# tsy935/eeg-gnn-ssl

Hardware: AMD Instinct MI355X
Metric: EEG clips/sec (60s, 19ch, K=2, 2-layer x64) fwd+bwd (higher is better)
Workload: dtype f32

## Files before the change

### eeg_gnn_ssl_amd/csrc/kernels_gemm_f.h

```cpp
#pragma once
#include "common.h"
#include "kernels_gemm_q.h"
#include "spec_launch.h"

namespace eeg {


__host__ __device__ constexpr int tnf_ndma(int FXT) { return (kTnfRC / 8) * (FXT + 10); }
__host__ __device__ constexpr int tnf_per(int FXT) { return (tnf_ndma(FXT) + 3) / 4; }

template <int FXT>
struct TnfRing {
    static constexpr int PER = tnf_per(FXT);
    const wbuf_t (&dsc)[PER];
    const int (&lofs)[PER];
    const unsigned (&vof)[PER];
    unsigned (&soff)[PER];
    const unsigned (&cstep)[PER];
};
template <int FXT, class LoadF, class MmaF>
__device__ __forceinline__ void tnf_ring(float* sm, const int Q, const TnfRing<FXT>& rg, LoadF load, MmaF mma) {
    constexpr int RC = kTnfRC, NS = tnf_ns(FXT), KS = RC / 2, PER = tnf_per(FXT), ST = tnf_stage_floats(FXT);
    int d_stage = 0;
    auto issue = [&]() __attribute__((always_inline)) {
        float* base = sm + d_stage * ST;
#pragma unroll
        for (int j = 0; j < PER; ++j) {
            wbuf_dma16(rg.dsc[j], base + rg.lofs[j], rg.vof[j], rg.soff[j]);
            rg.soff[j] += rg.cstep[j];
        }
        d_stage = d_stage + 1 == NS ? 0 : d_stage + 1;
    };
#pragma unroll
    for (int p = 0; p < NS - 1; ++p)
        if (p < Q) issue();
    int r_stage = 0;
    for (int q = 0; q < Q; ++q) {
        if (q + NS - 1 <= Q) vm_wait_barrier_n<(NS - 2) * PER>();
        else EEG_VM_WAIT_BARRIER(0);
#ifndef EEG_X_TNF_NODMA
        if (q + NS - 1 < Q) issue();
#endif
        const float* st = sm + r_stage * ST;
        load(IntC<0>(), st, 0);
#pragma unroll
        for (int ks = 0; ks < KS; ++ks) {
            if (ks & 1) {
                if (ks + 1 < KS) load(IntC<0>(), st, ks + 1);
                EEG_SCHED_FENCE();
                mma(IntC<1>());
            } else {
                if (ks + 1 < KS) load(IntC<1>(), st, ks + 1);
                EEG_SCHED_FENCE();
                mma(IntC<0>());
            }
            EEG_SCHED_FENCE();
        }
        r_stage = r_stage + 1 == NS ? 0 : r_stage + 1;
    }
}
__device__ __forceinline__ void tnf_store_tile(float* __restrict__ out, int ld, int f0, int c0, int fmax, int lane, const f32x16& t) {
    const int hh = lane >> 5, l32 = lane & 31;
#pragma unroll
    for (int v = 0; v < 16; ++v) {
        const int f = f0 + 8 * (v >> 2) + 4 * hh + (v & 3);
        if (f < fmax) out[(size_t)f * ld + c0 + l32] = t[v];
    }
}

template <int FXT, int S>
__device__ __forceinline__ void tnf_role(float* sm, const int Q, const int Fin, const int e, const int lane, const TnfRing<FXT>& rg,
                                         float* __restrict__ px, float* __restrict__ pg, float* __restrict__ pc) {
    constexpr int RC = kTnfRC, NXT = (FXT + 1) / 2;
    constexpr int RM = RC / 8, HI = RM * FXT * 256, RI = HI + RM * 512, YI = RI + RM * 512;
    constexpr int YX = 3 * S, YE = S == 0 ? 4 : 2;
    const int hh = lane >> 5, l32 = lane & 31;
    f32x16 ax[NXT][3], ah[2], ar;
#pragma unroll
    for (int v = 0; v < 16; ++v) {
#pragma unroll
        for (int a = 0; a < NXT; ++a)
#pragma unroll
            for (int c = 0; c < 3; ++c) ax[a][c][v] = 0.f;
        ah[0][v] = 0.f; ah[1][v] = 0.f; ar[v] = 0.f;
    }
    const int ox = hh * Fin + 32 * e + l32, oh = HI + hh * 64 + 32 * e + l32, orr = RI + hh * 64 + 32 * e + l32, oy = YI + hh * 192 + l32;
    float fx[2][NXT], fh[2], fr[2], fy[2][4];
    auto load = [&](auto PAR, const float* st, int ks) __attribute__((always_inline)) {
        constexpr int p = decltype(PAR)::value;
#pragma unroll
        for (int a = 0; a < NXT; ++a) fx[p][a] = st[ox + 2 * ks * Fin + 64 * a];
        fh[p] = st[oh + 2 * ks * 64];
        fr[p] = st[orr + 2 * ks * 64];
#pragma unroll
        for (int c = 0; c < 3; ++c) fy[p][c] = st[oy + 2 * ks * 192 + 32 * (YX + c)];
        fy[p][3] = st[oy + 2 * ks * 192 + 32 * YE];
    };
    auto mma = [&](auto PAR) __attribute__((always_inline)) {
        constexpr int p = decltype(PAR)::value;
#pragma unroll
        for (int a = 0; a < NXT; ++a)
#pragma unroll
#ifndef EEG_X_TNF_NOMFMA
            for (int c = 0; c < 3; ++c) ax[a][c] = mfma32(fx[p][a], fy[p][c], ax[a][c]);
#else
            for (int c = 0; c < 3; ++c) ax[a][c][0] += fx[p][a] * fy[p][c];
#endif
#ifndef EEG_X_TNF_NOMFMA
        ah[0] = mfma32(fh[p], S == 0 ? fy[p][0] : fy[p][3], ah[0]);
        ah[1] = mfma32(fh[p], S == 0 ? fy[p][1] : fy[p][0], ah[1]);
        ar = mfma32(fr[p], S == 0 ? fy[p][3] : fy[p][2], ar);
#else
        ah[0][0] += fh[p] * (S == 0 ? fy[p][0] : fy[p][3]);
        ah[1][0] += fh[p] * (S == 0 ? fy[p][1] : fy[p][0]);
        ar[0] += fr[p] * (S == 0 ? fy[p][3] : fy[p][2]);
#endif
    };
    tnf_ring<FXT>(sm, Q, rg, load, mma);
#pragma unroll
    for (int a = 0; a < NXT; ++a) {
        const int xe = e + 2 * a;
        if (xe >= FXT) continue;
#pragma unroll
        for (int c = 0; c < 3; ++c) tnf_store_tile(px, 192, 32 * xe, 32 * (YX + c), Fin, lane, ax[a][c]);
    }
    tnf_store_tile(pg, 128, 32 * e, 32 * (2 * S), 64, lane, ah[0]);
    tnf_store_tile(pg, 128, 32 * e, 32 * (2 * S + 1), 64, lane, ah[1]);
    tnf_store_tile(pc, 64, 32 * e, 32 * S, 64, lane, ar);
}

template <int S, int E>
__device__ __forceinline__ void tnf_role_r4(float* sm, const int Q, const int lane, const TnfRing<4>& rg,
                                            float* __restrict__ px, float* __restrict__ pg, float* __restrict__ pc) {
    constexpr int FXT = 4, Fin = 100, RC = kTnfRC, RM = RC / 8, HI = RM * FXT * 256, RI = HI + RM * 512, YI = RI + RM * 512;
    constexpr int YX = 3 * S, YE = S == 0 ? 4 : 2, NG = S == 0 ? 2 : 1, G0 = S == 0 ? 0 : 2;
    const int hh = lane >> 5, l32 = lane & 31;
    f32x16 t[8];
    f32x4 rem[2];
#pragma unroll
    for (int i = 0; i < 8; ++i)
#pragma unroll
        for (int v = 0; v < 16; ++v) t[i][v] = 0.f;
    rem[0] = rem[1] = (f32x4){0.f, 0.f, 0.f, 0.f};
    const int oxa = hh * Fin + (E == 0 ? 0 : 32) + l32, oxb = hh * Fin + 64 + l32;
    const int oh = HI + hh * 64 + 32 * E + l32, or0 = RI + hh * 64 + l32, oy = YI + hh * 192 + l32;
    const int oxr = 96 + (lane & 3), oyr = YI + lane;
    float fa[2][4], fy[2][4], ra[2][2], rb[2][2][2];
    auto load = [&](auto PAR, const float* st, int ks) __attribute__((always_inline)) {
        constexpr int p = decltype(PAR)::value;
        fa[p][0] = st[oxa + 2 * ks * Fin];
        fa[p][1] = st[E == 0 ? oxb + 2 * ks * Fin : oh + 2 * ks * 64];
        if (E == 0) fa[p][2] = st[oh + 2 * ks * 64];
        else { fa[p][2] = st[or0 + 2 * ks * 64]; fa[p][3] = st[or0 + 32 + 2 * ks * 64]; }
#pragma unroll
        for (int c = 0; c < 3; ++c) fy[p][c] = st[oy + 2 * ks * 192 + 32 * (YX + c)];
        if (E == 1 || S == 1) fy[p][3] = st[oy + 2 * ks * 192 + 32 * YE];
        if (E == 1) {
#pragma unroll
            for (int r = 0; r < 2; ++r) {
                ra[p][r] = st[(2 * ks + r) * Fin + oxr];
#pragma unroll
                for (int g = 0; g < NG; ++g) rb[p][r][g] = st[oyr + (2 * ks + r) * 192 + 64 * (G0 + g)];
            }
        }
    };
    auto mma = [&](auto PAR) __attribute__((always_inline)) {
        constexpr int p = decltype(PAR)::value;
        const float g0 = S == 0 ? fy[p][0] : fy[p][3], g1 = S == 0 ? fy[p][1] : fy[p][0];
#pragma unroll
        for (int c = 0; c < 3; ++c) t[c] = mfma32(fa[p][0], fy[p][c], t[c]);
        if (E == 0) {
#pragma unroll
            for (int c = 0; c < 3; ++c) t[3 + c] = mfma32(fa[p][1], fy[p][c], t[3 + c]);
            t[6] = mfma32(fa[p][2], g0, t[6]);
            t[7] = mfma32(fa[p][2], g1, t[7]);
        } else {
            const float cd = S == 0 ? fy[p][3] : fy[p][2];
            t[3] = mfma32(fa[p][1], g0, t[3]);
            t[4] = mfma32(fa[p][1], g1, t[4]);
            t[5] = mfma32(fa[p][2], cd, t[5]);
            t[6] = mfma32(fa[p][3], cd, t[6]);
#pragma unroll
            for (int r = 0; r < 2; ++r)
#pragma unroll
                for (int g = 0; g < NG; ++g) rem[g] = mfma4(ra[p][r], rb[p][r][g], rem[g]);
        }
    };
    tnf_ring<4>(sm, Q, rg, load, mma);
    if (E == 0) {
#pragma unroll
        for (int c = 0; c < 3; ++c) {
            tnf_store_tile(px, 192, 0, 32 * (YX + c), Fin, lane, t[c]);
            tnf_store_tile(px, 192, 64, 32 * (YX + c), Fin, lane, t[3 + c]);
        }
        tnf_store_tile(pg, 128, 0, 32 * (2 * S), 64, lane, t[6]);
        tnf_store_tile(pg, 128, 0, 32 * (2 * S + 1), 64, lane, t[7]);
    } else {
#pragma unroll
        for (int c = 0; c < 3; ++c) tnf_store_tile(px, 192, 32, 32 * (YX + c), Fin, lane, t[c]);
        tnf_store_tile(pg, 128, 32, 32 * (2 * S), 64, lane, t[3]);
        tnf_store_tile(pg, 128, 32, 32 * (2 * S + 1), 64, lane, t[4]);
        tnf_store_tile(pc, 64, 0, 32 * S, 64, lane, t[5]);
        tnf_store_tile(pc, 64, 32, 32 * S, 64, lane, t[6]);
#pragma unroll
        for (int g = 0; g < NG; ++g)
#pragma unroll
            for (int r = 0; r < 4; ++r) px[(size_t)(96 + r) * 192 + 64 * (G0 + g) + lane] = rem[g][r];
    }
}

template <int FXT>
__global__ __launch_bounds__(256, tnf_wgs_per_cu(FXT)) void gemm_tnf_kernel(const float* __restrict__ Xh, long long x_gstride, int Fin,
                                                         const float* __restrict__ Hh, long long h_gstride,
                                                         const float* __restrict__ RHh, const float* __restrict__ dY, int Sp, int spg, int rps,
                                                         float* __restrict__ part_x, float* __restrict__ part_g, float* __restrict__ part_c) {
    constexpr int RC = kTnfRC, RM = RC / 8, NDMA = tnf_ndma(FXT), PER = tnf_per(FXT), NX = RM * FXT, NH = RM * 2;
    constexpr int HI = NX * 256, RI = HI + NH * 256, YI = RI + NH * 256;
    EEG_DYN_SMEM(sm);
    const int tid = threadIdx.x, lane = tid & 63, w = wave_uniform(tid >> 6), e = w & 1, s = w >> 1;
    const int y = (int)blockIdx.x, i = y / spg, ls = y - i * spg;
    const int rbeg = ls * rps;
    int rend = rbeg + rps;
    if (rend > Sp) rend = Sp;
    const int Q = rend > rbeg ? (rend - rbeg) / RC : 0;
    wbuf_t dsc[PER];
    int lofs[PER];
    unsigned vof[PER], soff[PER], cstep[PER];
    const wbuf_t rx = make_wbuf(Xh + (size_t)i * x_gstride), rh = make_wbuf(Hh + (size_t)i * h_gstride);
    const wbuf_t rr = make_wbuf(RHh + (size_t)i * Sp * 64), ry = make_wbuf(dY + (size_t)i * Sp * 192);
#pragma unroll
    for (int j = 0; j < PER; ++j) {
        int d = w + 4 * j;
        if (d >= NDMA) d = NDMA - 1;
        if (d < NX) {
            dsc[j] = rx; lofs[j] = d * 256; cstep[j] = (unsigned)(RC * Fin) * 4u;
            soff[j] = (unsigned)(rbeg * Fin) * 4u;
            vof[j] = d * 1024 + lane * 16 < RC * Fin * 4 ? (unsigned)(d * 1024 + lane * 16) : 0u;
        } else if (d < NX + NH) {
            dsc[j] = rh; lofs[j] = HI + (d - NX) * 256; cstep[j] = RC * 64 * 4u;
            soff[j] = (unsigned)(rbeg * 64) * 4u; vof[j] = (unsigned)((d - NX) * 1024 + lane * 16);
        } else if (d < NX + 2 * NH) {
            dsc[j] = rr; lofs[j] = RI + (d - NX - NH) * 256; cstep[j] = RC * 64 * 4u;
            soff[j] = (unsigned)(rbeg * 64) * 4u; vof[j] = (unsigned)((d - NX - NH) * 1024 + lane * 16);
        } else {
            dsc[j] = ry; lofs[j] = YI + (d - NX - 2 * NH) * 256; cstep[j] = RC * 192 * 4u;
            soff[j] = (unsigned)(rbeg * 192) * 4u; vof[j] = (unsigned)((d - NX - 2 * NH) * 1024 + lane * 16);
        }
    }
    float* px = part_x + (size_t)y * Fin * 192;
    float* pg = part_g + (size_t)y * 64 * 128;
    float* pc = part_c + (size_t)y * 64 * 64;
    const TnfRing<FXT> rg{dsc, lofs, vof, soff, cstep};
#ifndef EEG_X_TNF_NOR4
    if constexpr (FXT == 4) {
        if (Fin == 100) {
            if (s == 0) { if (e == 0) tnf_role_r4<0, 0>(sm, Q, lane, rg, px, pg, pc); else tnf_role_r4<0, 1>(sm, Q, lane, rg, px, pg, pc); }
            else { if (e == 0) tnf_role_r4<1, 0>(sm, Q, lane, rg, px, pg, pc); else tnf_role_r4<1, 1>(sm, Q, lane, rg, px, pg, pc); }
            return;
        }
    }
#endif
    if (s == 0) tnf_role<FXT, 0>(sm, Q, Fin, e, lane, rg, px, pg, pc);
    else tnf_role<FXT, 1>(sm, Q, Fin, e, lane, rg, px, pg, pc);
}

template <int KQ, bool SWZ>
__global__ __launch_bounds__(256, 2) void gemm_nnf_kernel(const float* __restrict__ A, long long a_gstride, int K, int Sp, int G,
                                                         const float* __restrict__ Wr, unsigned w_gstride, float* __restrict__ C,
                                                         const float* __restrict__ bias, const float* __restrict__ gscale) {
    constexpr int NS = kNnfNS;
    EEG_DYN_SMEM(sm);
    const int tid = threadIdx.x, lane = tid & 63, w = wave_uniform(tid >> 6), rw = w & 1, cw = w >> 1, hh = lane >> 5, l32 = lane & 31;
    const int ST = nnf_stage_floats(K), CPG = ceil_div(Sp, 64), total = G * CPG;
    const int NPC = ceil_div(64 * K, 256), PER = ceil_div(NPC, 4);
    const int g0 = (int)(((long long)blockIdx.x * total) / gridDim.x), g1 = (int)(((long long)(blockIdx.x + 1) * total) / gridDim.x);
    const int Q = g1 - g0;
    if (tid < 4 * NS) sm[(tid >> 2) * ST + 64 * K + (tid & 3)] = 0.f;
    const unsigned lane_src = SWZ ? (unsigned)((lane >> 4) * 256 + (((lane & 15) ^ ((4 * w + (lane >> 4)) & 15)) << 4)) : (unsigned)lane * 16u;
    int d_g = g0, d_stage = 0, d_grp = -1;
    wbuf_t ra = make_wbuf_n(A, 0u);
    auto issue = [&]() __attribute__((always_inline)) {
        const int grp = d_g / CPG, lc = d_g - grp * CPG;
        if (grp != d_grp) { d_grp = grp; ra = make_wbuf_n(A + (size_t)grp * a_gstride, (unsigned)(Sp * K) * 4u); }
        float* base = sm + d_stage * ST;
        const unsigned cb = (unsigned)(lc * 64 * K) * 4u;
        for (int j = 0; j < PER; ++j) {
            int p = w + 4 * j;
            if (p >= NPC) p = NPC - 1;
            wbuf_dma16(ra, base + p * 256, cb + (unsigned)p * 1024u + lane_src, 0u);
        }
        d_stage = d_stage + 1 == NS ? 0 : d_stage + 1;
        ++d_g;
    };
    float wr[KQ][4][3];
    f32x16 acc[3];
    float binit[3] = {0.f, 0.f, 0.f};
    int c_grp = -1;
    wbuf_t rc = make_wbuf_n(C, 0u);
    const int row = 32 * rw + l32;
    const int a_row = row * K;
    const int ccol = 32 * 3 * cw + l32;
#pragma unroll 1
    for (int p = 0; p < NS - 1; ++p)
        if (p < Q) issue();
    int r_stage = 0;
#pragma unroll 1
    for (int q = 0; q < Q; ++q) {
        const int g = g0 + q, grp = g / CPG, lc = g - grp * CPG;
        if (grp != c_grp) {
            c_grp = grp;
            const wbuf_t rwt = make_wbuf(Wr + (size_t)grp * w_gstride);
#pragma unroll
            for (int kq = 0; kq < KQ; ++kq)
#pragma unroll
                for (int s = 0; s < 4; ++s)
#pragma unroll
                    for (int t = 0; t < 3; ++t) wr[kq][s][t] = wbuf_ld(rwt, (unsigned)(4 * hh * 192 + ccol), (unsigned)((8 * kq + s) * 192 + 32 * t));
            const float gs = bias != nullptr ? gscale[grp] : 0.f;
#pragma unroll
            for (int t = 0; t < 3; ++t) binit[t] = bias != nullptr ? gs * bias[ccol + 32 * t] : 0.f;
            rc = make_wbuf_n(C + (size_t)grp * Sp * 192, (unsigned)(Sp * 192) * 4u);
        }
        {
            int nd = Q - 1 - q;
            if (nd > NS - 2) nd = NS - 2;
            const int n = 48 * (q < NS - 1 ? q : NS - 1) + PER * nd;
            if (n >= 63) vm_wait_n<63>(); else if (n >= 55) vm_wait_n<55>(); else if (n >= 52) vm_wait_n<52>(); else if (n >= 48) vm_wait_n<48>();
            else if (n >= 14) vm_wait_n<14>(); else if (n >= 8) vm_wait_n<8>(); else if (n >= 7) vm_wait_n<7>(); else if (n >= 4) vm_wait_n<4>();
            else vm_wait_n<0>();
        }
#ifndef EEG_X_NNF_NOBAR
        EEG_LDS_BARRIER();
#endif
#ifndef EEG_X_NNF_NODMA
        if (q + NS - 1 < Q) issue();
#endif
        const float* st = sm + r_stage * ST;
#pragma unroll
        for (int t = 0; t < 3; ++t)
#pragma unroll
            for (int v = 0; v < 16; ++v) acc[t][v] = binit[t];
        f32x4 a4 = *reinterpret_cast<const f32x4*>(st + a_row + (SWZ ? ((hh ^ (row & 15)) << 2) : 4 * hh));
#pragma unroll
        for (int kq = 0; kq < KQ; ++kq) {
            f32x4 an = a4;
#ifndef EEG_X_NNF_NOLDS
            if (kq + 1 < KQ) an = *reinterpret_cast<const f32x4*>(st + a_row + (SWZ ? (((2 * (kq + 1) + hh) ^ (row & 15)) << 2) : 4 * (2 * (kq + 1) + hh)));
#endif
            EEG_SCHED_FENCE();
#pragma unroll
            for (int s = 0; s < 4; ++s)
#pragma unroll
                for (int t = 0; t < 3; ++t) acc[t] = mfma32(a4[s], wr[kq][s][t], acc[t]);
            EEG_SCHED_FENCE();
            a4 = an;
        }
        unsigned ob[4];
#pragma unroll
        for (int b = 0; b < 4; ++b) {
            ob[b] = (unsigned)((lc * 64 + 32 * rw + 4 * hh + 8 * b) * 192 + ccol);
            EEG_PIN(ob[b]);
        }
#pragma unroll
        for (int t = 0; t < 3; ++t)
#pragma unroll
#ifndef EEG_X_NNF_NOSTORE
            for (int v = 0; v < 16; ++v) wbuf_st1(rc, ob[v >> 2] + (unsigned)((v & 3) * 192 + 32 * t), 0u, acc[t][v]);
#else
            for (int v = 0; v < 16; ++v) { EEG_USE(acc[t][v]); (void)rc; }
#endif
        EEG_SCHED_FENCE();
        r_stage = r_stage + 1 == NS ? 0 : r_stage + 1;
    }
}


template <int NT>
__global__ __launch_bounds__(256, 2) void gemm_dxf_kernel(const float* __restrict__ dYh, int Sp, int S, int Nrt, const float* __restrict__ Wtq,
                                                         unsigned w_gstride, const float* __restrict__ basis, float* __restrict__ dX) {
    const int N = NT > 0 ? NT : Nrt;
    constexpr int NS = kDxfNS, ST = kDxfStage, RB = kDxfRows, PER = 6;
    EEG_DYN_SMEM(sm);
    const int tid = threadIdx.x, lane = tid & 63, w = wave_uniform(tid >> 6), lr = lane & 15, lg = lane >> 4;
    const int r0 = (int)blockIdx.x * RB;
    unsigned src[PER];
#pragma unroll
    for (int j = 0; j < PER; ++j) {
        const int P = 64 * (w + 4 * j) + lane, row = P / 48, slot = P - row * 48;
        const int unit = (slot & ~15) | ((slot & 15) ^ (row & 15));
        src[j] = (unsigned)((r0 + row) * 768 + unit * 16);
    }
    int d_i = 0, d_stage = 0;
    auto issue = [&]() __attribute__((always_inline)) {
        const wbuf_t ra = make_wbuf_n(dYh + (size_t)d_i * Sp * 192, (unsigned)(Sp * 192) * 4u);
        float* base = sm + d_stage * ST;
#pragma unroll
        for (int j = 0; j < PER; ++j) wbuf_dma16(ra, base + (w + 4 * j) * 256, src[j], 0u);
        d_stage = d_stage + 1 == NS ? 0 : d_stage + 1;
        if (d_i + 1 < N) ++d_i;
    };
    f32x4 acc[kDxfMaxN][2];
#pragma unroll
    for (int j = 0; j < kDxfMaxN; ++j) acc[j][0] = acc[j][1] = (f32x4){0.f, 0.f, 0.f, 0.f};
    f32x4 wq[12];
    const unsigned wl = (unsigned)(w * 64 + lane) * 4u;
    static_assert(kDxfNS == 3, "the queue discipline below is written for two images in flight");
    issue();
    issue();
    EEG_SCHED_FENCE();
    {
        const wbuf_t rw0 = make_wbuf(Wtq);
#pragma unroll
        for (int c = 0; c < 12; ++c) wq[c] = wbuf_ld4(rw0, wl, (unsigned)(c * 4 * 256));
    }
    vm_wait_n<PER + 12>();
    int r_stage = 0;
    const int a_row = lr * 192;
#pragma unroll 1
    for (int i = 0; i < N; ++i) {
        EEG_LDS_BARRIER();
#ifndef EEG_X_DXF_NODMA
        issue();
#endif
        const wbuf_t rwn = make_wbuf(Wtq + (size_t)(i + 1 < N ? i + 1 : i) * w_gstride);
        const float* st = sm + r_stage * ST;
        float uu[kDxfMaxN];
#pragma unroll
        for (int j = 0; j < kDxfMaxN; ++j) uu[j] = (NT > 0 ? j < NT : j < N) ? basis[j * N + i] : 0.f;
        f32x4 t0 = {0.f, 0.f, 0.f, 0.f}, t1 = {0.f, 0.f, 0.f, 0.f};
        auto frag_off = [&](int c) __attribute__((always_inline)) {
            const int u = 4 * c + lg;
            return a_row + (((u & ~15) | ((u & 15) ^ lr)) << 2);
        };
        f32x4 fa[2][2];
        fa[0][0] = *reinterpret_cast<const f32x4*>(st + frag_off(0));
        fa[0][1] = *reinterpret_cast<const f32x4*>(st + 16 * 192 + frag_off(0));
#pragma unroll
        for (int c = 0; c < 12; ++c) {
            if (c + 1 < 12) {
                fa[(c + 1) & 1][0] = *reinterpret_cast<const f32x4*>(st + frag_off(c + 1));
                fa[(c + 1) & 1][1] = *reinterpret_cast<const f32x4*>(st + 16 * 192 + frag_off(c + 1));
            }
            EEG_SCHED_FENCE();
#pragma unroll
            for (int e = 0; e < 4; ++e) {
                t0 = mfma16(wq[c][e], fa[c & 1][0][e], t0);
                t1 = mfma16(wq[c][e], fa[c & 1][1][e], t1);
            }
            EEG_SCHED_FENCE();
#ifndef EEG_X_DXF_NOW
            wq[c] = wbuf_ld4(rwn, wl, (unsigned)(c * 4 * 256));
#endif
            EEG_SCHED_FENCE();
        }
#pragma unroll
        for (int j = 0; j < kDxfMaxN; ++j)
            if (NT > 0 ? j < NT : j < N) {
                acc[j][0] += t0 * uu[j];
                acc[j][1] += t1 * uu[j];
            }
        r_stage = r_stage + 1 == NS ? 0 : r_stage + 1;
    }
    const wbuf_t rx = make_wbuf_n(dX, (unsigned)(S * N * 64) * 4u);
#pragma unroll
    for (int t = 0; t < 2; ++t) {
        const unsigned rb = (unsigned)((r0 + 16 * t + lr) * N * 64 + 16 * w + 4 * lg);
#pragma unroll
        for (int j = 0; j < kDxfMaxN; ++j)
            if (j < N) wbuf_st4(rx, rb + (unsigned)(j * 64), 0u, acc[j][t]);
    }
}

}
```

### eeg_gnn_ssl_amd/csrc/spec_common.h

```cpp
#pragma once
#include "common.h"
#include "nnq_order.h"

namespace eeg {

constexpr int kSpecTc = kMaxM * 32, kSpecInfo = 32, kSpecCsum = 32;
__host__ __device__ constexpr int spec_basis_floats(int N) { return N * N + kSpecTc + kSpecInfo + kSpecCsum; }
__host__ __device__ constexpr int spec_csum_offset(int N) { return N * N + kSpecTc + kSpecInfo; }
__host__ __device__ constexpr int spec_rows(int S) { return round_up(S, 16); }
constexpr int kSpecSweeps = 12;

struct SpecPack {
    int Fin, H, M, N;
    int nch_x, nct_x, nch_t, nct_t;
    size_t sxq, sxq_stride, sxtq, sxtq_stride, sxr, sxr_stride, total;
};
__host__ __device__ inline SpecPack make_spec_pack(int Fin, int H, int M, int N) {
    SpecPack p;
    p.Fin = Fin; p.H = H; p.M = M; p.N = N;
    p.nch_x = make_nnq_order(1, Fin).nch; p.nct_x = 3 * H / 16;
    p.nch_t = make_nnq_order(1, 3 * H).nch; p.nct_t = round_up(Fin, 16) / 16;
    p.sxq_stride = (size_t)p.nch_x * p.nct_x * 256;
    p.sxtq_stride = (size_t)p.nch_t * p.nct_t * 256;
    p.sxq = 0;
    p.sxtq = p.sxq + p.sxq_stride * N;
    p.sxr = p.sxtq + p.sxtq_stride * N;
    p.sxr_stride = (size_t)round_up(Fin, 8) * 3 * H;
    p.total = p.sxr + p.sxr_stride * N;
    return p;
}
struct SpecFoldJob {
    const float* part;
    int spg, K, O, nblocks;
};
struct SpecFoldJobs {
    SpecFoldJob j[3];
    const float* basis;
    int N;
};
__host__ __device__ inline size_t spec_fold_lds_bytes(int M, int nsplit_max) { return 256 * 16 + (size_t)M * nsplit_max * sizeof(float); }
template <int MM>
__device__ __forceinline__ void spec_fold_block_m(int block, const SpecFoldJob& jb, int kind, const float* __restrict__ basis, int N,
                                                   int acc_flag, int Fin, int H, int M, float* __restrict__ dWg, float* __restrict__ dWc) {
    EEG_DYN_SMEM(sm);
    float4 (*red)[16] = reinterpret_cast<float4 (*)[16]>(sm);
    float* tcl = sm + 256 * 4;
    const int O = jb.O;
    const size_t total = (size_t)jb.K * O;
    const int g = threadIdx.x >> 4, q = threadIdx.x & 15;
    const size_t idx4 = ((size_t)block * 16 + q) * 4;
    const float* tc = basis + N * N;
    const int nsplit = N * jb.spg;
    for (int e = threadIdx.x; e < M * nsplit; e += 256) {
        const int m = e / nsplit, sp = e - m * nsplit;
        tcl[e] = tc[m * 32 + sp / jb.spg];
    }
    __syncthreads();
    float4 a[MM];
#pragma unroll
    for (int m = 0; m < MM; ++m) a[m] = make_float4(0.f, 0.f, 0.f, 0.f);
    if (idx4 < total) {
        constexpr int UN = 8;
        for (int base = g; base < nsplit; base += 16 * UN) {
            float4 v[UN];
#pragma unroll
            for (int u = 0; u < UN; ++u) {
                const int sp = base + 16 * u;
                v[u] = sp < nsplit ? *reinterpret_cast<const float4*>(jb.part + (size_t)sp * total + idx4) : make_float4(0.f, 0.f, 0.f, 0.f);
            }
#pragma unroll
            for (int u = 0; u < UN; ++u) {
                const int sp = base + 16 * u < nsplit ? base + 16 * u : 0;
#pragma unroll
                for (int m = 0; m < MM; ++m) {
                    if (m < M) {
                        const float t = tcl[m * nsplit + sp];
                        a[m].x = fmaf(t, v[u].x, a[m].x); a[m].y = fmaf(t, v[u].y, a[m].y);
                        a[m].z = fmaf(t, v[u].z, a[m].z); a[m].w = fmaf(t, v[u].w, a[m].w);
                    }
                }
            }
        }
    }
#pragma unroll
    for (int m = 0; m < MM; ++m) {
        if (m >= M) break;
        __syncthreads();
        red[g][q] = a[m];
        __syncthreads();
        if (g == 0 && idx4 < total) {
            float4 sum = red[0][q];
#pragma unroll
            for (int u = 1; u < 16; ++u) {
                const float4 v = red[u][q];
                sum.x += v.x; sum.y += v.y; sum.z += v.z; sum.w += v.w;
            }
            const float sv[4] = {sum.x, sum.y, sum.z, sum.w};
#pragma unroll
            for (int e = 0; e < 4; ++e) {
                const size_t idx = idx4 + e;
                const int f = (int)(idx / O), o = (int)(idx % O);
                float* dst;
                if (kind == 0) dst = o < 2 * H ? &dWg[((size_t)f * M + m) * (2 * H) + o] : &dWc[((size_t)f * M + m) * H + (o - 2 * H)];
                else if (kind == 1) dst = &dWg[((size_t)(Fin + f) * M + m) * (2 * H) + o];
                else dst = &dWc[((size_t)(Fin + f) * M + m) * H + o];
                *dst = acc_flag ? *dst + sv[e] : sv[e];
            }
        }
    }
}
__device__ __forceinline__ void spec_fold_block(int block, const SpecFoldJob& jb, int kind, const float* __restrict__ basis, int N,
                                                int acc_flag, int Fin, int H, int M, float* __restrict__ dWg, float* __restrict__ dWc) {
    if (M <= 4) spec_fold_block_m<4>(block, jb, kind, basis, N, acc_flag, Fin, H, M, dWg, dWc);
    else spec_fold_block_m<kMaxM>(block, jb, kind, basis, N, acc_flag, Fin, H, M, dWg, dWc);
}

}
```

Baseline: 137,000.

## Overlap GEMM output stores with MFMA and double-buffer spectral fold loads

In the NNF GEMM, the stores of each output column tile are spread between the MFMA instructions of the next tile, and the last tile of one iteration is stored during the following iteration, so global writes overlap compute. In the dX kernel, the final image's stores are interleaved with its MFMAs when N is compile-time. The spectral fold kernel double-buffers its partial loads across iterations, issues them before LDS setup, and reduces all M outputs in one barrier pass instead of one barrier pair per m. This adds LDS usage (M times the reduction buffer) and register pressure from the extra load buffers and the carried accumulator.

```diff
diff --git a/eeg_gnn_ssl_amd/csrc/kernels_gemm_f.h b/eeg_gnn_ssl_amd/csrc/kernels_gemm_f.h
--- a/eeg_gnn_ssl_amd/csrc/kernels_gemm_f.h
+++ b/eeg_gnn_ssl_amd/csrc/kernels_gemm_f.h
@@ -294,12 +294,26 @@
     };
     float wr[KQ][4][3];
     f32x16 acc[3];
+#pragma unroll
+    for (int v = 0; v < 16; ++v) acc[2][v] = 0.f;
     float binit[3] = {0.f, 0.f, 0.f};
     int c_grp = -1;
-    wbuf_t rc = make_wbuf_n(C, 0u);
+    wbuf_t rc = make_wbuf_n(C, 0u), rcp = rc;
+    unsigned obp[4] = {0u, 0u, 0u, 0u};
     const int row = 32 * rw + l32;
     const int a_row = row * K;
     const int ccol = 32 * 3 * cw + l32;
+    auto store1 = [&](const wbuf_t& r, const unsigned (&o)[4], const f32x16& tile, int t, int v) __attribute__((always_inline)) {
+#ifndef EEG_X_NNF_NOSTORE
+        wbuf_st1(r, o[v >> 2] + (unsigned)((v & 3) * 192 + 32 * t), 0u, tile[v]);
+#else
+        EEG_USE(tile[v]); (void)r; (void)o;
+#endif
+    };
+    auto frag = [&](const float* st, int kq) __attribute__((always_inline)) {
+        return *reinterpret_cast<const f32x4*>(st + a_row + (SWZ ? (((2 * kq + hh) ^ (row & 15)) << 2) : 4 * (2 * kq + hh)));
+    };
+    constexpr int NM = 4 * KQ;
 #pragma unroll 1
     for (int p = 0; p < NS - 1; ++p)
         if (p < Q) issue();
@@ -311,11 +325,11 @@
             c_grp = grp;
             const wbuf_t rwt = make_wbuf(Wr + (size_t)grp * w_gstride);
 #pragma unroll
-            for (int kq = 0; kq < KQ; ++kq)
-#pragma unroll
-                for (int s = 0; s < 4; ++s)
-#pragma unroll
-                    for (int t = 0; t < 3; ++t) wr[kq][s][t] = wbuf_ld(rwt, (unsigned)(4 * hh * 192 + ccol), (unsigned)((8 * kq + s) * 192 + 32 * t));
+            for (int t = 0; t < 3; ++t)
+#pragma unroll
+                for (int kq = 0; kq < KQ; ++kq)
+#pragma unroll
+                    for (int s = 0; s < 4; ++s) wr[kq][s][t] = wbuf_ld(rwt, (unsigned)(4 * hh * 192 + ccol), (unsigned)((8 * kq + s) * 192 + 32 * t));
             const float gs = bias != nullptr ? gscale[grp] : 0.f;
 #pragma unroll
             for (int t = 0; t < 3; ++t) binit[t] = bias != nullptr ? gs * bias[ccol + 32 * t] : 0.f;
@@ -335,26 +349,8 @@
 #ifndef EEG_X_NNF_NODMA
         if (q + NS - 1 < Q) issue();
 #endif
+        EEG_SCHED_FENCE();
         const float* st = sm + r_stage * ST;
-#pragma unroll
-        for (int t = 0; t < 3; ++t)
-#pragma unroll
-            for (int v = 0; v < 16; ++v) acc[t][v] = binit[t];
-        f32x4 a4 = *reinterpret_cast<const f32x4*>(st + a_row + (SWZ ? ((hh ^ (row & 15)) << 2) : 4 * hh));
-#pragma unroll
-        for (int kq = 0; kq < KQ; ++kq) {
-            f32x4 an = a4;
-#ifndef EEG_X_NNF_NOLDS
-            if (kq + 1 < KQ) an = *reinterpret_cast<const f32x4*>(st + a_row + (SWZ ? (((2 * (kq + 1) + hh) ^ (row & 15)) << 2) : 4 * (2 * (kq + 1) + hh)));
-#endif
-            EEG_SCHED_FENCE();
-#pragma unroll
-            for (int s = 0; s < 4; ++s)
-#pragma unroll
-                for (int t = 0; t < 3; ++t) acc[t] = mfma32(a4[s], wr[kq][s][t], acc[t]);
-            EEG_SCHED_FENCE();
-            a4 = an;
-        }
         unsigned ob[4];
 #pragma unroll
         for (int b = 0; b < 4; ++b) {
@@ -362,16 +358,38 @@
             EEG_PIN(ob[b]);
         }
 #pragma unroll
-        for (int t = 0; t < 3; ++t)
-#pragma unroll
-#ifndef EEG_X_NNF_NOSTORE
-            for (int v = 0; v < 16; ++v) wbuf_st1(rc, ob[v >> 2] + (unsigned)((v & 3) * 192 + 32 * t), 0u, acc[t][v]);
-#else
-            for (int v = 0; v < 16; ++v) { EEG_USE(acc[t][v]); (void)rc; }
-#endif
-        EEG_SCHED_FENCE();
+        for (int t = 0; t < 3; ++t) {
+#pragma unroll
+            for (int v = 0; v < 16; ++v) acc[t][v] = binit[t];
+            f32x4 a4 = frag(st, 0);
+#pragma unroll
+            for (int kq = 0; kq < KQ; ++kq) {
+                f32x4 an = a4;
+#ifndef EEG_X_NNF_NOLDS
+                if (kq + 1 < KQ) an = frag(st, kq + 1);
+#endif
+                EEG_SCHED_FENCE();
+#pragma unroll
+                for (int s = 0; s < 4; ++s) {
+                    const int m = 4 * kq + s;
+                    acc[t] = mfma32(a4[s], wr[kq][s][t], acc[t]);
+#pragma unroll
+                    for (int j = m * 16 / NM; j < (m + 1) * 16 / NM; ++j) {
+                        if (t == 0) store1(rcp, obp, acc[2], 2, j);
+                        else store1(rc, ob, acc[t - 1], t - 1, j);
+                    }
+                    EEG_SCHED_FENCE();
+                }
+                a4 = an;
+            }
+        }
+        rcp = rc;
+#pragma unroll
+        for (int b = 0; b < 4; ++b) obp[b] = ob[b];
         r_stage = r_stage + 1 == NS ? 0 : r_stage + 1;
     }
+#pragma unroll
+    for (int j = 0; j < 16; ++j) store1(rcp, obp, acc[2], 2, j);
 }
 
 
@@ -416,8 +434,13 @@
     vm_wait_n<PER + 12>();
     int r_stage = 0;
     const int a_row = lr * 192;
+    auto frag_off = [&](int c) __attribute__((always_inline)) {
+        const int u = 4 * c + lg;
+        return a_row + (((u & ~15) | ((u & 15) ^ lr)) << 2);
+    };
+    const int n_loop = NT > 0 ? N - 1 : N;
 #pragma unroll 1
-    for (int i = 0; i < N; ++i) {
+    for (int i = 0; i < n_loop; ++i) {
         EEG_LDS_BARRIER();
 #ifndef EEG_X_DXF_NODMA
         issue();
@@ -428,10 +451,6 @@
 #pragma unroll
         for (int j = 0; j < kDxfMaxN; ++j) uu[j] = (NT > 0 ? j < NT : j < N) ? basis[j * N + i] : 0.f;
         f32x4 t0 = {0.f, 0.f, 0.f, 0.f}, t1 = {0.f, 0.f, 0.f, 0.f};
-        auto frag_off = [&](int c) __attribute__((always_inline)) {
-            const int u = 4 * c + lg;
-            return a_row + (((u & ~15) | ((u & 15) ^ lr)) << 2);
-        };
         f32x4 fa[2][2];
         fa[0][0] = *reinterpret_cast<const f32x4*>(st + frag_off(0));
         fa[0][1] = *reinterpret_cast<const f32x4*>(st + 16 * 192 + frag_off(0));
@@ -462,8 +481,43 @@
         r_stage = r_stage + 1 == NS ? 0 : r_stage + 1;
     }
     const wbuf_t rx = make_wbuf_n(dX, (unsigned)(S * N * 64) * 4u);
-#pragma unroll
-    for (int t = 0; t < 2; ++t) {
+    if constexpr (NT > 0) {
+        constexpr int NN = NT;
+        const int i = N - 1;
+        EEG_LDS_BARRIER();
+        const float* st = sm + r_stage * ST;
+        float uu[kDxfMaxN];
+#pragma unroll
+        for (int j = 0; j < kDxfMaxN; ++j) uu[j] = (NT > 0 ? j < NT : j < N) ? basis[j * N + i] : 0.f;
+#pragma unroll
+        for (int t = 0; t < 2; ++t) {
+            const unsigned rbp = (unsigned)((r0 + lr) * N * 64 + 16 * w + 4 * lg);
+            f32x4 tt = {0.f, 0.f, 0.f, 0.f};
+            f32x4 fa[2];
+            fa[0] = *reinterpret_cast<const f32x4*>(st + 16 * 192 * t + frag_off(0));
+#pragma unroll
+            for (int c = 0; c < 12; ++c) {
+                if (c + 1 < 12) fa[(c + 1) & 1] = *reinterpret_cast<const f32x4*>(st + 16 * 192 * t + frag_off(c + 1));
+                EEG_SCHED_FENCE();
+#pragma unroll
+                for (int e = 0; e < 4; ++e) {
+                    tt = mfma16(wq[c][e], fa[c & 1][e], tt);
+                    if (t == 1) {
+#pragma unroll
+                        for (int j = (4 * c + e) * NN / 48; j < (4 * c + e + 1) * NN / 48; ++j)
+                            if (j < N) wbuf_st4(rx, rbp + (unsigned)(j * 64), 0u, acc[j][0]);
+                        EEG_SCHED_FENCE();
+                    }
+                }
+                EEG_SCHED_FENCE();
+            }
+#pragma unroll
+            for (int j = 0; j < kDxfMaxN; ++j)
+                if (NT > 0 ? j < NT : j < N) acc[j][t] += tt * uu[j];
+        }
+    }
+#pragma unroll
+    for (int t = NT > 0 ? 1 : 0; t < 2; ++t) {
         const unsigned rb = (unsigned)((r0 + 16 * t + lr) * N * 64 + 16 * w + 4 * lg);
 #pragma unroll
         for (int j = 0; j < kDxfMaxN; ++j)
diff --git a/eeg_gnn_ssl_amd/csrc/spec_common.h b/eeg_gnn_ssl_amd/csrc/spec_common.h
--- a/eeg_gnn_ssl_amd/csrc/spec_common.h
+++ b/eeg_gnn_ssl_amd/csrc/spec_common.h
@@ -38,74 +38,88 @@
     const float* basis;
     int N;
 };
-__host__ __device__ inline size_t spec_fold_lds_bytes(int M, int nsplit_max) { return 256 * 16 + (size_t)M * nsplit_max * sizeof(float); }
+__host__ __device__ inline size_t spec_fold_lds_bytes(int M, int nsplit_max) { return (size_t)M * 256 * 16 + (size_t)M * (32 + nsplit_max) * sizeof(float); }
 template <int MM>
 __device__ __forceinline__ void spec_fold_block_m(int block, const SpecFoldJob& jb, int kind, const float* __restrict__ basis, int N,
                                                    int acc_flag, int Fin, int H, int M, float* __restrict__ dWg, float* __restrict__ dWc) {
     EEG_DYN_SMEM(sm);
-    float4 (*red)[16] = reinterpret_cast<float4 (*)[16]>(sm);
-    float* tcl = sm + 256 * 4;
+    float4 (*red)[16][16] = reinterpret_cast<float4 (*)[16][16]>(sm);
+    float* tcr = sm + M * 256 * 4;
+    float* tcl = tcr + M * 32;
     const int O = jb.O;
     const size_t total = (size_t)jb.K * O;
     const int g = threadIdx.x >> 4, q = threadIdx.x & 15;
     const size_t idx4 = ((size_t)block * 16 + q) * 4;
     const float* tc = basis + N * N;
     const int nsplit = N * jb.spg;
+    const bool on = idx4 < total;
+    constexpr int UN = 8;
+    float4 v0[UN], v1[UN];
+    auto request = [&](float4 (&v)[UN], int base) __attribute__((always_inline)) {
+#pragma unroll
+        for (int u = 0; u < UN; ++u) {
+            const int sp = base + 16 * u;
+            v[u] = on && sp < nsplit ? *reinterpret_cast<const float4*>(jb.part + (size_t)sp * total + idx4) : make_float4(0.f, 0.f, 0.f, 0.f);
+        }
+    };
+    const float tcv = (int)threadIdx.x < M * 32 ? tc[threadIdx.x] : 0.f;
+    request(v0, g);
+    request(v1, g + 16 * UN);
+    if ((int)threadIdx.x < M * 32) tcr[threadIdx.x] = tcv;
+    EEG_LDS_BARRIER();
     for (int e = threadIdx.x; e < M * nsplit; e += 256) {
         const int m = e / nsplit, sp = e - m * nsplit;
-        tcl[e] = tc[m * 32 + sp / jb.spg];
+        tcl[e] = tcr[m * 32 + sp / jb.spg];
     }
-    __syncthreads();
+    EEG_LDS_BARRIER();
     float4 a[MM];
 #pragma unroll
     for (int m = 0; m < MM; ++m) a[m] = make_float4(0.f, 0.f, 0.f, 0.f);
-    if (idx4 < total) {
-        constexpr int UN = 8;
-        for (int base = g; base < nsplit; base += 16 * UN) {
-            float4 v[UN];
+    auto consume = [&](const float4 (&v)[UN], int base) __attribute__((always_inline)) {
 #pragma unroll
-            for (int u = 0; u < UN; ++u) {
-                const int sp = base + 16 * u;
-                v[u] = sp < nsplit ? *reinterpret_cast<const float4*>(jb.part + (size_t)sp * total + idx4) : make_float4(0.f, 0.f, 0.f, 0.f);
-            }
+        for (int u = 0; u < UN; ++u) {
+            const int sp = base + 16 * u < nsplit ? base + 16 * u : 0;
 #pragma unroll
-            for (int u = 0; u < UN; ++u) {
-                const int sp = base + 16 * u < nsplit ? base + 16 * u : 0;
-#pragma unroll
-                for (int m = 0; m < MM; ++m) {
-                    if (m < M) {
-                        const float t = tcl[m * nsplit + sp];
-                        a[m].x = fmaf(t, v[u].x, a[m].x); a[m].y = fmaf(t, v[u].y, a[m].y);
-                        a[m].z = fmaf(t, v[u].z, a[m].z); a[m].w = fmaf(t, v[u].w, a[m].w);
-                    }
+            for (int m = 0; m < MM; ++m) {
+                if (m < M) {
+                    const float t = tcl[m * nsplit + sp];
+                    a[m].x = fmaf(t, v[u].x, a[m].x); a[m].y = fmaf(t, v[u].y, a[m].y);
+                    a[m].z = fmaf(t, v[u].z, a[m].z); a[m].w = fmaf(t, v[u].w, a[m].w);
                 }
             }
         }
+    };
+    if (on) {
+        for (int base = g; base < nsplit; base += 32 * UN) {
+            consume(v0, base);
+            request(v0, base + 32 * UN);
+            if (base + 16 * UN < nsplit) consume(v1, base + 16 * UN);
+            request(v1, base + 48 * UN);
+        }
     }
 #pragma unroll
-    for (int m = 0; m < MM; ++m) {
-        if (m >= M) break;
-        __syncthreads();
-        red[g][q] = a[m];
-        __syncthreads();
-        if (g == 0 && idx4 < total) {
-            float4 sum = red[0][q];
+    for (int m = 0; m < MM; ++m)
+        if (m < M) red[m][g][q] = a[m];
+    __syncthreads();
+    if (g < M && on) {
+        const int m = g;
+        float4 sum = red[m][0][q];
 #pragma unroll
-            for (int u = 1; u < 16; ++u) {
-                const float4 v = red[u][q];
-                sum.x += v.x; sum.y += v.y; sum.z += v.z; sum.w += v.w;
-            }
-            const float sv[4] = {sum.x, sum.y, sum.z, sum.w};
+        for (int u = 1; u < 16; ++u) {
+            const float4 v = red[m][u][q];
+            sum.x += v.x; sum.y += v.y; sum.z += v.z; sum.w += v.w;
+        }
+        const float sv[4] = {sum.x, sum.y, sum.z, sum.w};
+        const int f0 = (int)(idx4 / O), o0 = (int)(idx4 - (size_t)f0 * O);
 #pragma unroll
-            for (int e = 0; e < 4; ++e) {
-                const size_t idx = idx4 + e;
-                const int f = (int)(idx / O), o = (int)(idx % O);
-                float* dst;
-                if (kind == 0) dst = o < 2 * H ? &dWg[((size_t)f * M + m) * (2 * H) + o] : &dWc[((size_t)f * M + m) * H + (o - 2 * H)];
-                else if (kind == 1) dst = &dWg[((size_t)(Fin + f) * M + m) * (2 * H) + o];
-                else dst = &dWc[((size_t)(Fin + f) * M + m) * H + o];
-                *dst = acc_flag ? *dst + sv[e] : sv[e];
-            }
+        for (int e = 0; e < 4; ++e) {
+            int f = f0, o = o0 + e;
+            if (o >= O) { o -= O; ++f; }
+            float* dst;
+            if (kind == 0) dst = o < 2 * H ? &dWg[((size_t)f * M + m) * (2 * H) + o] : &dWc[((size_t)f * M + m) * H + (o - 2 * H)];
+            else if (kind == 1) dst = &dWg[((size_t)(Fin + f) * M + m) * (2 * H) + o];
+            else dst = &dWc[((size_t)(Fin + f) * M + m) * H + o];
+            *dst = acc_flag ? *dst + sv[e] : sv[e];
         }
     }
 }
```

Result: no change. 138,200, median of 6 (+0.9%).
